# leekwoon/nav-gym

Measured on AMD Instinct MI355X. Metric: env steps/sec (whole node), 4096 envs x 1081-beam lidar, higher is better.
Workload: dtype f32

## Files before the change

### nav-gym_amd/csrc/kernels_step.hpp

```cpp

struct StepShared {
    double rp[3];
    double old_rp[3];
    double act[2];
    float lx, ly, lth;
    int steps_now;
    double cT, sT;
    int i0, j0;
    int nseg, ndisc;
    int rescan;
    int respawn;
    float t1;
    float r_all;
    unsigned long long step_key;
    unsigned long long rescan_key;
    int next_chunk;
    int park_count, park_next;
    int pair_done;
    int term;
    double wave_ratio[kMaxWaves];
};
struct PedShared {
    double *ax, *ay, *avx, *avy;
    float (*seg)[4];
    float (*disc)[2];
    float* info;
};
__host__ __device__ inline size_t ped_lds_bytes(int N) { return (size_t)144 * N + 32; }
__host__ __device__ inline size_t ped_pair_bytes(int N) { return ((size_t)(N * (N - 1) / 2 + N) * sizeof(double2) + 15) & ~(size_t)15; }
__device__ __forceinline__ PedShared ped_lds_carve(char* base, int N) {
    PedShared ps;
    double* d = (double*)base;
    ps.ax = d; ps.ay = d + (N + 1); ps.avx = d + 2 * (N + 1); ps.avy = d + 3 * (N + 1);
    float* f = (float*)(d + 4 * (N + 1));
    ps.seg = (float(*)[4])f;
    ps.disc = (float(*)[2])(f + 16 * N);
    ps.info = f + 20 * N;
    return ps;
}
struct Prims { const float (*seg)[4]; const float (*disc)[2]; float* info; };

template <int BLOCK>
__device__ __forceinline__ void finish_beams(const navsim_config& c, const StepShared& sh, const Prims pr,
                                             const double* __restrict__ tab, const float2* __restrict__ dir,
                                             const float* __restrict__ rng, float* __restrict__ rng_rw,
                                             const float* __restrict__ thr, const float* __restrict__ dthr,
                                             float* __restrict__ obs_row, int n_hist, float noise_std,
                                             uint64_t noise_key, uint64_t genv, int& crash, int& discomfort);

__device__ __forceinline__ void sfm_pair(const navsim_config& c, double xi, double yi, double vxi, double vyi,
                                         double xj, double yj, double vxj, double vyj, double& fx, double& fy) {
    fx = 0.0; fy = 0.0;
    double dxx = xj - xi, dyy = yj - yi;
    double dist = sqrt(dxx * dxx + dyy * dyy);
    if (dist < 1e-9) return;
    double ddx = dxx / dist, ddy = dyy / dist;
    double ivx = c.sfm_lambda * (vxi - vxj) + ddx;
    double ivy = c.sfm_lambda * (vyi - vyj) + ddy;
    double il = sqrt(ivx * ivx + ivy * ivy);
    if (il < 1e-9) return;
    double idx = ivx / il, idy = ivy / il;
    double theta = nv::atan2_(idx * ddy - idy * ddx, idx * ddx + idy * ddy);
    double Bq = c.sfm_gamma * il;
    double a1 = c.sfm_n_prime * Bq * theta;
    double a2 = c.sfm_n * Bq * theta;
    double fv = -nv::exp_neg(-dist / Bq - a1 * a1);
    double sgn = (theta > 0.0) ? 1.0 : ((theta < 0.0) ? -1.0 : 0.0);
    double fa = -sgn * nv::exp_neg(-dist / Bq - a2 * a2);
    fx = fv * idx + fa * (-idy);
    fy = fv * idy + fa * idx;
// ... 236 lines not shown
            if (mask_lane(inval)) raw = field.load(px, py);
            occ = (occ & ~inval) | (inval & mask_of(field.occupied(raw)));
            d = mask_sel(inval, field.decode_nz(raw, px, py), d);
        }
    } else {
        typename Field::raw_t raw = field.load(px, py);
        occ = live & mask_of(field.occupied(raw));
        d = field.decode_nz(raw, px, py);
    }
    hit |= occ;
    const float tn = t + march_step<RULE>(d);
    const lanemask_t go = live & ~occ;
    t = mask_sel(go, tn, t);
    active = go & mask_flt(tn, max_range);
}

constexpr int kIntRangeMaxSide = 1448;
__host__ __device__ __forceinline__ bool int_range_ok(int H, int W) { return H <= kIntRangeMaxSide && W <= kIntRangeMaxSide; }
__device__ __forceinline__ float hit_range_int(int ix, int iy) {
    return nv::sqrt_small_int((float)(__mul24(ix, ix) + __mul24(iy, iy)));
}
template <int RULE>
__device__ __forceinline__ float ray_result(lanemask_t hit, bool int_range, int i0, int j0, float x0, float y0, float dx, float dy,
                                            float t, float miss) {
    const int px = (int)march_pos<RULE>(x0, dx, t), py = (int)march_pos<RULE>(y0, dy, t);
    float r;
    if (int_range) {
        r = hit_range_int(px - i0, py - j0);
    } else {
        const float xd = (float)px - x0, yd = (float)py - y0;
        r = sqrtf(xd * xd + yd * yd);
    }
    return mask_sel(hit, r, miss);
}

#ifndef NAVSIM_PARK_LANES
#define NAVSIM_PARK_LANES 16
#endif
#ifndef NAVSIM_PAIR_SHARE_MIN_BLOCK
#define NAVSIM_PAIR_SHARE_MIN_BLOCK 512
#endif
constexpr int kParkLanesMax = NAVSIM_PARK_LANES;
#ifndef NAVSIM_PARK_LANES_PEDS
#define NAVSIM_PARK_LANES_PEDS 16
#endif
#ifdef NAVSIM_PARK_512
__host__ __device__ constexpr bool step_parks(int block, bool peds) { return (block == 256 && (!peds || NAVSIM_PARK_LANES_PEDS > 0)) || (block == 512 && !peds); }
#else
__host__ __device__ constexpr bool step_parks(int block, bool peds) { return block == 256 && (!peds || NAVSIM_PARK_LANES_PEDS > 0); }
#endif
__host__ __device__ inline size_t park_lds_bytes(int B, int park_lanes, bool peds) {
    return (((size_t)((B + 63) / 64) * park_lanes * (peds ? 2 : 16)) + 15) & ~(size_t)15;
}
__device__ __forceinline__ int lanes_below(lanemask_t m) {
    return (int)__builtin_amdgcn_mbcnt_hi((unsigned)(m >> 32), __builtin_amdgcn_mbcnt_lo((unsigned)m, 0u));
}

template <int BLOCK, typename Field, bool TO_LDS, int RULE, int RECT>
__device__ __forceinline__ void scan_beams_pred(const navsim_config& c, StepShared& sh,
                                                const Field& field, const uint4* __restrict__ rects,
                                                const double* __restrict__ tab,
                                                const Prims pr, float2* __restrict__ dir_lds, float* __restrict__ rng_lds,
                                                float4* __restrict__ park, const int park_lanes,
                                                const float* __restrict__ thr, const float* __restrict__ dthr,
                                                float* __restrict__ obs_row, int n_hist, float noise_std,
                                                uint64_t noise_key, uint64_t genv,
                                                int& crash, int& discomfort, bool prepare_prims = true) {
    const int B = c.n_beams, S = c.n_scan_stack, H = c.map_h, W = c.map_w;
    const float max_range = march_limit(H, W, c.range_max, c.resolution);
    const float res = (float)c.resolution;
    const float rmax = (float)c.range_max;
    const double step = nv::linspace_step(c);
    const int i0 = sh.i0, j0 = sh.j0;
    const float x0 = (float)i0, y0 = (float)j0;
    const bool int_range = int_range_ok(H, W);
    const float lx = sh.lx, ly = sh.ly;
    const int nseg = sh.nseg, ndisc = sh.ndisc;
    const unsigned uW = (unsigned)W, uH = (unsigned)H;
    const unsigned tpr = (unsigned)((W + 7) >> kRectShift);
    const float t1 = sh.t1, r_all = sh.r_all;
    const uint64_t nkey = (noise_std > 0.0f) ? nv::noise_stream(c.seed, genv, noise_key) : 0;
    int cr = 0, dc = 0;
    auto finish = [&](int k, float dx, float dy, float rr) {
        if (TO_LDS) {
            rng_lds[k] = rr * res;
            dir_lds[k] = make_float2(dx, dy);
            return;
        }
        rr = rr * res;
        for (int p = 0; p < nseg; ++p)
            nv::seg_merge(rr, lx, ly, dx, dy, pr.seg[p][0], pr.seg[p][1], pr.seg[p][2], pr.seg[p][3]);
        for (int p = 0; p < ndisc; ++p)
            nv::circle_merge(rr, lx, ly, dx, dy, pr.disc[p][0], pr.disc[p][1], nv::kLegRadius);
        rr = rr < 0.0f ? 0.0f : rr;
        rr = rr > rmax ? rmax : rr;
        if (noise_std > 0.0f && rr != rmax)
            rr = rr + noise_std * nv::gauss_noise(nkey, (uint32_t)k);
        cr |= (rr < thr[k]);
        dc |= (rr < dthr[k]);
        obs_row[(size_t)(S - 1) * B + k] = rr;
        for (int j = 0; j < S - 1; ++j)
            if (S - 1 - j > n_hist) obs_row[(size_t)j * B + k] = rr;
    };
    const float miss = (r_all >= 0.0f) ? r_all : max_range;
    if constexpr (TO_LDS) { if (prepare_prims) prims_prepare<BLOCK>(c, sh, pr); }
    constexpr bool kPark = step_parks(BLOCK, TO_LDS);
    int own_chunk = 0;
    const int lane = (int)threadIdx.x & 63;
    for (;;) {
        int chunk = 0;
        if (BLOCK > 64) {
            if (lane == 0) chunk = atomicAdd(&sh.next_chunk, 1);
            chunk = __builtin_amdgcn_readfirstlane(chunk);
        } else {
            chunk = own_chunk++;
        }
        if (chunk * 64 >= B) break;
        const int k = chunk * 64 + lane;
        const bool valid = k < B;
        float dx, dy;
        beam_dir_k(c, tab, valid ? k : B - 1, step, (double)sh.lth, sh.cT, sh.sT, dx, dy);
        float t = t1;
        lanemask_t active = mask_of(valid & (r_all < 0.0f));
        lanemask_t hit = 0;
        if constexpr (!kPark) {
            while (active != 0)
                probe_round<Field, RULE, RECT>(field, (const char*)rects, tpr, x0, y0, dx, dy, uW, uH, max_range, t, active, hit);
            if (valid) finish(k, dx, dy, ray_result<RULE>(hit, int_range, i0, j0, x0, y0, dx, dy, t, miss));
        } else {
            while ((int)__builtin_popcountll(active) > park_lanes)
                probe_round<Field, RULE, RECT>(field, (const char*)rects, tpr, x0, y0, dx, dy, uW, uH, max_range, t, active, hit);
            const bool marching = mask_lane(active);
            if (active != 0) {
                int base = 0;
                if (lane == 0) base = atomicAdd(&sh.park_count, (int)__builtin_popcountll(active));
                base = __builtin_amdgcn_readfirstlane(base);
                if (marching) {
                    if constexpr (TO_LDS) {
                        ((unsigned short*)park)[base + lanes_below(active)] = (unsigned short)k;
                        rng_lds[k] = t;
                        dir_lds[k] = make_float2(dx, dy);
                    } else {
                        park[base + lanes_below(active)] = make_float4(__int_as_float(k), t, dx, dy);
                    }
                }
            }
            if (valid & !marching) finish(k, dx, dy, ray_result<RULE>(hit, int_range, i0, j0, x0, y0, dx, dy, t, miss));
        }
    }
    if constexpr (kPark) __syncthreads();
    const int n_parked = kPark ? sh.park_count : 0;
    for (;;) {
        if (!kPark || n_parked == 0) break;
        int g = 0;
        if (lane == 0) g = atomicAdd(&sh.park_next, 64);
        g = __builtin_amdgcn_readfirstlane(g);
        if (g >= n_parked) break;
        const bool valid = g + lane < n_parked;
        int k;
        float t, dx, dy;
        if constexpr (TO_LDS) {
            k = (int)((const unsigned short*)park)[valid ? g + lane : g];
            t = rng_lds[k];
            const float2 d = dir_lds[k];
            dx = d.x; dy = d.y;
        } else {
            const float4 r = park[valid ? g + lane : g];
            k = __float_as_int(r.x);
            t = r.y; dx = r.z; dy = r.w;
        }
        lanemask_t active = mask_of(valid);
        lanemask_t hit = 0;
        while (active != 0)
            probe_round<Field, RULE, RECT>(field, (const char*)rects, tpr, x0, y0, dx, dy, uW, uH, max_range, t, active, hit);
        if (valid) finish(k, dx, dy, ray_result<RULE>(hit, int_range, i0, j0, x0, y0, dx, dy, t, miss));
    }
    if (TO_LDS) {
        __syncthreads();
        finish_beams<BLOCK>(c, sh, pr, tab, dir_lds, rng_lds, rng_lds, thr, dthr, obs_row, n_hist, noise_std,
                            noise_key, genv, cr, dc);
    }
    crash = cr;
    discomfort = dc;
}

__device__ __forceinline__ int ped_pop_waypoints(const double* wp, int head, int nw, const double (&pp)[3]) {
    while (head + 1 < nw) {
        double ddx = pp[0] - wp[2 * head], ddy = pp[1] - wp[2 * head + 1];
        if (sqrt(ddx * ddx + ddy * ddy) < 1.0) ++head;
        else break;
    }
    return head;
}
__device__ __forceinline__ void ped_pair_index(int t, int n, int& i, int& j) {
    const int n_pp = n * (n - 1) / 2;
    if (t < n_pp) {
        i = 0;
        int rem = t;
        while (rem >= n - 1 - i) { rem -= n - 1 - i; ++i; }
        j = i + 1 + rem;
    } else {
        i = t - n_pp; j = n;
    }
}
__device__ __forceinline__ void ped_pair_term(const navsim_config& c, const PedShared& ps, double2* pair, int n, int t) {
    int i, j;
    ped_pair_index(t, n, i, j);
    double fx, fy;
    sfm_pair(c, ps.ax[i], ps.ay[i], ps.avx[i], ps.avy[i], ps.ax[j], ps.ay[j], ps.avx[j], ps.avy[j], fx, fy);
    pair[t] = make_double2(fx, fy);
}
template <typename Field>
__device__ __forceinline__ void ped_sfm_step(const navsim_config& c, const Field& field, const PedShared& ps,
                                             const double2* pair, int n, int i, double vpref, const double* wp, double dt,
                                             double (&pp)[3], double (&pvel)[2]) {
    double ex = wp[0] - ps.ax[i], ey = wp[1] - ps.ay[i];
    double L = sqrt(ex * ex + ey * ey);
    if (L > 1e-9) { ex = ex / L; ey = ey / L; } else { ex = 0.0; ey = 0.0; }
    double fdx = (vpref * ex - ps.avx[i]) / c.sfm_tau;
    double fdy = (vpref * ey - ps.avy[i]) / c.sfm_tau;
    double fsx = 0.0, fsy = 0.0;
    {
        int slot = i - 1;
        for (int j = 0; j < i; ++j) {
            const double2 f = pair[slot];
            fsx -= f.x;
            fsy -= f.y;
            slot += n - 2 - j;
        }
        slot = i * (n - 1) - i * (i - 1) / 2;
        for (int j = i + 1; j < n; ++j, ++slot) {
            const double2 f = pair[slot];
            fsx += f.x;
// ... 520 lines not shown
            }
        }
        const double th = th_old + a1 * dt;
        const double th_new = reset_only ? th_old : nv::mod_2pi(th);
        const float lth = (float)th_new;
        const double ang = (l0 == 0) ? th_old : ((l0 == 1) ? th : (double)lth);
        double sn, cs;
        nv::sincos(ang, sn, cs);
        const int w0 = kPhase0Thread & 63;
        const double s0 = __shfl(sn, w0), c0 = __shfl(cs, w0), s1 = __shfl(sn, w0 + 1), c1 = __shfl(cs, w0 + 1);
        const double sT = __shfl(sn, w0 + 2), cT = __shfl(cs, w0 + 2);
        if (l0 == 0) {
            sh.old_rp[0] = rp_g[0]; sh.old_rp[1] = rp_g[1]; sh.old_rp[2] = th_old;
            sh.nseg = 0; sh.ndisc = 0; sh.rescan = 0; sh.respawn = 0; sh.term = 0;
            if constexpr (INSTALL) {
                if (pending && !in->lone) {
                    if (in->late) in->late[e] = 0;
                    if (in->late_next) in->late_next[e] = 0;
                    if (in->late_prev && in->late_prev[e]) {
                        sh.respawn = 4;
                        stage_request(in->stage.episode, in->mark, e, st.episode[e] + 1);
                        if (st.counters) atomicAdd(&st.counters[NAVSIM_COUNTER_REGEN_LATE], 1ull);
                    } else if (in->ready) {
                        const bool lng = c.regen_min_steps <= 0 || st.done_steps[e] >= c.regen_min_steps;
                        const bool rdy = stage_ready(in->ready, e) == (long long)st.episode[e];
                        if (lng && rdy) sh.respawn = 3;
                        else {
                            if (lng && in->late) in->late[e] = 1;
                            stage_request(in->stage.episode, in->mark, e, st.episode[e] + 1);
                        }
                        if (st.counters)
                            atomicAdd(&st.counters[lng ? (rdy ? NAVSIM_COUNTER_REGEN_SERVED : NAVSIM_COUNTER_REGEN_LATE) : NAVSIM_COUNTER_REGEN_SHORT], 1ull);
                    }
                }
            }
            if (!reset_only) {
                const int64_t steps_now = st.steps[e] + 1;
                st.steps[e] = steps_now;
                sh.steps_now = (int)steps_now;
                sh.act[0] = a0; sh.act[1] = a1;
                double p[3] = {sh.old_rp[0], sh.old_rp[1], sh.old_rp[2]};
                nv::set_vel_with(p, a0, a1, dt, c.axle_offset, s0, c0, s1, c1, nullptr);
                sh.rp[0] = p[0]; sh.rp[1] = p[1]; sh.rp[2] = p[2];
            } else {
                sh.rp[0] = sh.old_rp[0]; sh.rp[1] = sh.old_rp[1]; sh.rp[2] = sh.old_rp[2];
            }
            sh.lx = (float)sh.rp[0]; sh.ly = (float)sh.rp[1]; sh.lth = (float)sh.rp[2];
            nv::xy_to_ij_f32(sh.lx, sh.ly, c, sh.i0, sh.j0);
            sh.sT = sT; sh.cT = cT;
            first_probe<RULE>(field, sh.i0, sh.j0, (float)((long long)c.map_h * c.map_w), sh.t1, sh.r_all);
            sh.step_key = (unsigned long long)st.episode[e] * 0x100000000ULL +
                          (unsigned long long)(reset_only ? 0 : st.steps[e]) * 2ULL;
            sh.rescan_key = sh.step_key + 1;
            sh.next_chunk = 0; sh.park_count = 0; sh.park_next = 0; sh.pair_done = 0;
        }
    }
    __syncthreads();
    if constexpr (INSTALL) {
        if (pending && sh.respawn == 3) {
            install_arena<BLOCK>(c, st, io, *in, e, obs_row);
            install_publish(*in, st, e);
            return;
        }
        if (pending && sh.respawn == 4) return;
    }

    NAVSIM_STAMP(1);
    if constexpr (PEDS) {
        double2* pair = (double2*)(dyn_lds + ((dyn_lds_bytes + 15u) & ~15u) + ((ped_lds_bytes(N) + 15) & ~(size_t)15));
#ifdef NAVSIM_PAIR_SHARE_ALL
        constexpr int kPairWaves = (BLOCK >= NAVSIM_PAIR_SHARE_MIN_BLOCK) ? 4 : 1;
#else
        constexpr int kPairWaves = (INSTALL && BLOCK >= NAVSIM_PAIR_SHARE_MIN_BLOCK) ? 4 : 1;
#endif
        const bool pair_shared = PINL && kPairWaves > 1 && ped_advance && c.ped_model == NAVSIM_PED_SFM;
        if constexpr (PINL && kPairWaves > 1) {
            if (pair_shared && tid < kPairWaves * 64) ped_pair_share(c, ps, pair, n, tid, kPairWaves, &sh.pair_done);
        }
        if (tid < 64) {
            const int lane = tid;
            if constexpr (PINL) {
                if (ped_advance)
                    ped_advance_wave<Field>(c, st, field, e, n, lane, is_ped, pq, dt, genv, (uint64_t)st.steps[e], ps, pair,
                                            ped_head, ped_nw, pp, pvel, &sh.pair_done, pair_shared ? kPairWaves : 1);
            }
            if (reset_only && is_ped) {
                st.ped_dist[pq * 3] = 0.0; st.ped_dist[pq * 3 + 1] = 0.0; st.ped_dist[pq * 3 + 2] = 0.0;
                st.ped_prev_yaw[pq] = nv::wrap_pi(pp[2]);
            }
            if (is_ped) {
                float dist3[3];
                if (reset_only) { dist3[0] = dist3[1] = dist3[2] = 0.0f; }
                else { dist3[0] = (float)st.ped_dist[pq * 3]; dist3[1] = (float)st.ped_dist[pq * 3 + 1];
                       dist3[2] = (float)st.ped_dist[pq * 3 + 2]; }
                if (st.ped_has_legs[pq] && c.lidar_legs) {
                    float cc[4];
                    nv::leg_centres((float)pp[0], (float)pp[1], (float)pp[2], dist3[0], dist3[1], dist3[2], cc);
                    int q = atomicAdd(&sh.ndisc, 2);
                    ps.disc[q][0] = cc[0]; ps.disc[q][1] = cc[1];
                    ps.disc[q + 1][0] = cc[2]; ps.disc[q + 1][1] = cc[3];
                } else {
                    const double fpx[4] = {0.22, -0.22, -0.22, 0.22};
                    const double fpy[4] = {0.19, 0.19, -0.19, -0.19};
                    double s, cs;
                    nv::sincos(pp[2], s, cs);
                    float vx[4], vy[4];
#pragma unroll
                    for (int v = 0; v < 4; ++v) {
                        vx[v] = (float)((cs * fpx[v] - s * fpy[v]) + pp[0]);
                        vy[v] = (float)((s * fpx[v] + cs * fpy[v]) + pp[1]);
                    }
                    int q = atomicAdd(&sh.nseg, 4);
#pragma unroll
                    for (int v = 0; v < 4; ++v) {
                        int w = (v + 1) & 3;
                        ps.seg[q + v][0] = vx[v]; ps.seg[q + v][1] = vy[v];
                        ps.seg[q + v][2] = vx[w]; ps.seg[q + v][3] = vy[w];
                    }
                }
            }
            wave_lds_sync();
            prims_prepare<64>(c, sh, prims);
        }
    }

    NAVSIM_STAMP(2);
    if (kMarchPrio == 2 || base_prio == 2) __builtin_amdgcn_s_setprio(2);
    else if (base_prio == 1) __builtin_amdgcn_s_setprio(1);
    else __builtin_amdgcn_s_setprio(0);
    int n_hist = reset_only ? 0 : st.n_hist[e];
    int crash = 0, discomfort = 0;
    const uint64_t step_key = sh.step_key;
    float4* park = (float4*)dyn_lds;
    char* scan_lds = dyn_lds + park_lds_bytes(B, park_lanes, PEDS);
    float2* dir_lds = (float2*)scan_lds;
    float* rng_lds = (float*)(scan_lds + sizeof(float2) * (size_t)B);
    scan_beams_pred<BLOCK, Field, PEDS, RULE, RECT>(c, sh, field, rects, st.beam_table, prims, dir_lds, rng_lds, park, park_lanes, st.scan_threshold,
                                                         st.scan_discomfort, obs_row, n_hist, noise_std, step_key, genv, crash, discomfort, false);

    NAVSIM_STAMP(3);
    bool restart_next = false;
    if (!reset_only) {
        crash = __syncthreads_or(crash);
        discomfort = __syncthreads_or(discomfort);
        double rmin = 1.0e300;
        if (discomfort && !crash) {
            for (int k = tid; k < B; k += BLOCK)
            {
                double ratio = nv::discomfort_ratio((double)obs_row[(size_t)(S - 1) * B + k],
                                                    st.scan_threshold[k], st.scan_discomfort[k]);
                rmin = ratio < rmin ? ratio : rmin;
            }
            rmin = wave_min_f64(rmin);
            if ((tid & 63) == 0) sh.wave_ratio[tid >> 6] = rmin;
            __syncthreads();
        }
        NAVSIM_STAMP(4);
        if (tid == 0) {
            if (discomfort && !crash)
                for (int w = 1; w < (BLOCK + 63) / 64; ++w) rmin = sh.wave_ratio[w] < rmin ? sh.wave_ratio[w] : rmin;
            double prev_xy[2] = {pv_g[0], pv_g[1]};
            double pose[2] = {sh.rp[0], sh.rp[1]};
            double vel[2] = {pa_g[0], pa_g[1]};
            double goal[2] = {goal_g[0], goal_g[1]};
            nv::RewardOut o = nv::reward_scalar(c, prev_xy, pose, vel, goal, crash != 0, discomfort != 0, rmin);
            if constexpr (kFeat) {
                if (c.max_episode_steps > 0) {
                    const bool trunc = !o.done && sh.steps_now >= c.max_episode_steps;
                    if (io.truncated) io.truncated[e] = (uint8_t)trunc;
                    if (trunc) o.done = 1;
                }
            }
            io.reward[e] = o.reward;
            io.done[e] = (uint8_t)o.done;
            if constexpr (INSTALL) { if (in->late) in->late[e] = 0; if (in->late_next) in->late_next[e] = 0; }
            io.is_success[e] = o.success;
            io.is_crash[e] = o.crash;
            io.distance[e] = o.distance;
            const bool restart = o.done && c.auto_reset != NAVSIM_AUTORESET_NONE && c.n_spawn > 0;
            if (restart && c.auto_reset == NAVSIM_AUTORESET_SAME_STEP) {
                if (kFeat && io.final_obs) {
                    const bool crashed = o.crash != 0.0f;
                    const double tx = crashed ? pv_g[0] : sh.rp[0], ty = crashed ? pv_g[1] : sh.rp[1];
                    const double tyaw = nv::wrap_pi(crashed ? pv_g[2] : sh.rp[2]);
                    float* ft = io.final_obs + (size_t)e * D + (size_t)S * B;
                    ft[0] = (float)pv_g[0]; ft[1] = (float)pv_g[1];
                    ft[2] = (float)tx; ft[3] = (float)ty;
                    ft[4] = (float)pa_g[0]; ft[5] = (float)pa_g[1];
                    ft[6] = (float)tyaw;
                    if (io.final_goals) {
                        float* fg = io.final_goals + 4 * (size_t)e;
                        fg[0] = (float)tx; fg[1] = (float)ty; fg[2] = (float)goal_g[0]; fg[3] = (float)goal_g[1];
                    }
                    sh.term = crashed ? 2 : 1;
                }
                uint64_t h = nv::hash4(c.seed, genv, (uint64_t)st.episode[e], 0x5eedULL);
                int idx = (int)(h % (uint64_t)c.n_spawn);
                const double* sp = st.spawn_pose + ((size_t)e * c.n_spawn + idx) * 3;
                const double* sg = st.spawn_goal + ((size_t)e * c.n_spawn + idx) * 2;
                sh.rp[0] = sp[0]; sh.rp[1] = sp[1]; sh.rp[2] = sp[2];
                goal_g[0] = sg[0]; goal_g[1] = sg[1];
#ifndef NAVSIM_DIAG_NO_DONE_STEPS
                if (st.done_steps) st.done_steps[e] = sh.steps_now;
#endif
                st.episode[e] += 1;
                st.steps[e] = 0;
                sh.rescan_key = (unsigned long long)st.episode[e] * 0x100000000ULL;
                sh.respawn = 1; sh.rescan = c.defer_reset_scan ? 0 : 1;
                if constexpr (INSTALL) if (in->ready) {
                    const bool lng = c.regen_min_steps <= 0 || st.done_steps[e] >= c.regen_min_steps;
                    const bool rdy = stage_ready(in->ready, e) == (long long)st.episode[e];
                    if (lng && rdy) { sh.respawn = 3; sh.rescan = 0; }
                    else if (lng && in->late) in->late[e] = 1;
                    if (st.counters)
                        atomicAdd(&st.counters[lng ? (rdy ? NAVSIM_COUNTER_REGEN_SERVED : NAVSIM_COUNTER_REGEN_LATE) : NAVSIM_COUNTER_REGEN_SHORT], 1ull);
                    if (!(lng && rdy)) stage_request(in->stage.episode, in->mark, e, st.episode[e] + 1);
                }
            } else {
                restart_next = kFeat && restart;
                if (o.crash != 0.0f) {
                    sh.rp[0] = pv_g[0]; sh.rp[1] = pv_g[1]; sh.rp[2] = pv_g[2];
                    sh.rescan = 1;
                }
            }
#ifdef NAVSIM_DIAG_NO_RESCAN
            sh.rescan = 0;
#endif
            if constexpr (!kFeat) {
                if (sh.rescan) {
                    sh.next_chunk = 0; sh.park_count = 0; sh.park_next = 0;
                    sh.lx = (float)sh.rp[0]; sh.ly = (float)sh.rp[1]; sh.lth = (float)sh.rp[2];
                    nv::xy_to_ij_f32(sh.lx, sh.ly, c, sh.i0, sh.j0);
                    nv::sincos((double)sh.lth, sh.sT, sh.cT);
                    first_probe<RULE>(field, sh.i0, sh.j0, (float)((long long)c.map_h * c.map_w), sh.t1, sh.r_all);
                }
            }
        }
        __syncthreads();
        if constexpr (!kFeat) {
            if (sh.rescan) {
                if (sh.respawn) n_hist = 0;
                int c2, d2;
                scan_beams_pred<BLOCK, Field, PEDS, RULE, RECT>(c, sh, field, rects, st.beam_table, prims, dir_lds, rng_lds, park, park_lanes, st.scan_threshold,
                                                                     st.scan_discomfort, obs_row, n_hist, noise_std, sh.rescan_key, genv, c2, d2);
            }
        } else {
            float* final_row = io.final_obs ? io.final_obs + (size_t)e * D : nullptr;
            const int term = sh.term;
            if (term == 1) {
                for (int j = 0; j < S; ++j) {
                    const bool old = j < S - 1 && S - 1 - j <= n_hist;
                    for (int k = tid; k < B; k += BLOCK)
                        final_row[(size_t)j * B + k] = old ? obs_prev[(size_t)(j + 1) * B + k] : obs_row[(size_t)(S - 1) * B + k];
                }
                __syncthreads();
            }
            for (int pass = (term == 2) ? 0 : 1; pass < 2; ++pass) {
                if (pass == 1 && !sh.rescan) break;
                if (tid == 0) {
                    const double* at = (pass == 0) ? pv_g : sh.rp;
                    sh.next_chunk = 0; sh.park_count = 0; sh.park_next = 0;
                    sh.lx = (float)at[0]; sh.ly = (float)at[1]; sh.lth = (float)at[2];
                    nv::xy_to_ij_f32(sh.lx, sh.ly, c, sh.i0, sh.j0);
                    nv::sincos((double)sh.lth, sh.sT, sh.cT);
                    first_probe<RULE>(field, sh.i0, sh.j0, (float)((long long)c.map_h * c.map_w), sh.t1, sh.r_all);
                }
                __syncthreads();
                if (pass == 1 && sh.respawn) n_hist = 0;
                int c2, d2;
                scan_beams_pred<BLOCK, Field, PEDS, RULE, RECT>(c, sh, field, rects, st.beam_table, prims, dir_lds, rng_lds, park, park_lanes, st.scan_threshold,
                                                                     st.scan_discomfort, pass == 0 ? final_row : obs_row, n_hist, noise_std,
                                                                     pass == 0 ? step_key + 1 : sh.rescan_key, genv, c2, d2);
                if (pass == 0) {
                    for (int j = 0; j < S - 1; ++j)
                        if (S - 1 - j <= n_hist)
                            for (int k = tid; k < B; k += BLOCK) final_row[(size_t)j * B + k] = obs_prev[(size_t)(j + 1) * B + k];
                    __syncthreads();
                }
            }
        }
    }

    NAVSIM_STAMP(5);
    if (kMarchPrio != 0 && base_prio < kMarchPrio) {
        if (base_prio == 1) __builtin_amdgcn_s_setprio(1);
        else __builtin_amdgcn_s_setprio(0);
    }
    const bool fresh = reset_only || sh.respawn;
    if (!fresh && obs_prev) {
        for (int j = 0; j < S - 1; ++j)
            if (S - 1 - j <= n_hist)
                for (int k = tid; k < B; k += BLOCK) obs_row[(size_t)j * B + k] = obs_prev[(size_t)(j + 1) * B + k];
    }
    if (tid == 0) {
        float* tail = obs_row + (size_t)S * B;
        double yaw = nv::wrap_pi(sh.rp[2]);
        double pxy0 = fresh ? sh.rp[0] : pv_g[0];
        double pxy1 = fresh ? sh.rp[1] : pv_g[1];
        double v0 = fresh ? 0.0 : pa_g[0], v1 = fresh ? 0.0 : pa_g[1];
        tail[0] = (float)pxy0; tail[1] = (float)pxy1;
        tail[2] = (float)sh.rp[0]; tail[3] = (float)sh.rp[1];
        tail[4] = (float)v0; tail[5] = (float)v1;
        tail[6] = (float)yaw;
        if (io.achieved_goal) { io.achieved_goal[2 * e] = (float)sh.rp[0]; io.achieved_goal[2 * e + 1] = (float)sh.rp[1]; }
        if (io.desired_goal) { io.desired_goal[2 * e] = (float)goal_g[0]; io.desired_goal[2 * e + 1] = (float)goal_g[1]; }
        rp_g[0] = sh.rp[0]; rp_g[1] = sh.rp[1]; rp_g[2] = sh.rp[2];
        if (fresh) { pa_g[0] = 0.0; pa_g[1] = 0.0; st.n_hist[e] = (S - 1 < 1) ? S - 1 : 1; }
        else       { pa_g[0] = sh.act[0]; pa_g[1] = sh.act[1]; st.n_hist[e] = (n_hist + 1 < S - 1) ? n_hist + 1 : S - 1; }
        if (reset_only) st.steps[e] = 0;
        pv_g[0] = sh.rp[0]; pv_g[1] = sh.rp[1]; pv_g[2] = yaw;
        if (restart_next) {
            uint64_t h = nv::hash4(c.seed, genv, (uint64_t)st.episode[e], 0x5eedULL);
            int idx = (int)(h % (uint64_t)c.n_spawn);
            const double* sp = st.spawn_pose + ((size_t)e * c.n_spawn + idx) * 3;
            const double* sg = st.spawn_goal + ((size_t)e * c.n_spawn + idx) * 2;
            rp_g[0] = sp[0]; rp_g[1] = sp[1]; rp_g[2] = sp[2];
            goal_g[0] = sg[0]; goal_g[1] = sg[1];
            if (st.done_steps) st.done_steps[e] = sh.steps_now;
            st.episode[e] += 1;
            st.steps[e] = 0;
            if constexpr (INSTALL) {
                if (in->late_next && in->ready) {
                    const bool lng = c.regen_min_steps <= 0 || sh.steps_now >= c.regen_min_steps;
// ... 191 lines not shown
```

### nav-gym_amd/csrc/navsim_step_inst.hip

```cpp
#include "preamble.hpp"

#if !defined(NAVSIM_INST_BLOCK) || !defined(NAVSIM_INST_PEDS)
#error "compile with -DNAVSIM_INST_BLOCK=64|256|512|1024 -DNAVSIM_INST_PEDS=0|1 (csrc/Makefile)"
#endif

namespace {
#include "kernels_field.hpp"
#include "kernels_rect.hpp"
#include "kernels_plan.hpp"
#include "kernels_regen_dev.hpp"
#include "kernels_step.hpp"
}
#include "step_plan.hpp"

namespace {

template <typename Kernel, typename... Args>
int launch(Kernel kernel, const StepLaunch& l, int blocks, int block, size_t lds, const Args&... args) {
    if (allow_lds((const void*)kernel, lds) != NAVSIM_OK) return NAVSIM_E_UNSUPPORTED;
    if (l.prepare_only) return NAVSIM_OK;
    kernel<<<blocks, block, lds, l.stream>>>(args...);
    return NAVSIM_OK;
}

template <int BLOCK, bool PEDS, typename Field, int RECT, int RULE, bool PINL>
int launch_step_pinl(const navsim_config* c, const navsim_state* st, const navsim_step_io* io, const StepLaunch& l, const StepPlan& p) {
    constexpr bool kPacked = !std::is_same<Field, FieldF32>::value;
    const unsigned scan = (unsigned)step_lds_scan_bytes(c, p.park);
    const int blocks = l.grid > 0 ? l.grid : c->n_envs;
    if constexpr (PEDS && PINL) {
        if (l.part == kStepPartReplan) {
            const size_t pl = plan_lds(c->map_h / 5, c->map_w / 5), lds = p.lds > pl ? p.lds : pl;
            if (l.install) {
                if constexpr (kPacked)
                    return launch(navsim_step_replan_install_kernel<BLOCK, Field, RULE, RECT>, l, l.grid + c->n_envs, BLOCK, lds,
                                  *c, *st, *io, *l.install, scan, p.park, p.rect_off, l.grid, l.max_queries);
                return NAVSIM_E_UNSUPPORTED;
            }
            return launch(navsim_step_replan_kernel<BLOCK, Field, RULE, RECT>, l, l.grid + c->n_envs, BLOCK, lds,
                          *c, *st, *io, scan, p.park, p.rect_off, l.grid, l.max_queries);
        }
        if (l.part == NAVSIM_STEP_DUE)
            return launch(navsim_step_due_kernel<BLOCK, Field, RULE, RECT>, l, blocks, BLOCK, p.lds, *c, *st, *io, scan, p.park, p.rect_off);
    }
    if constexpr (PINL == PEDS && kPacked) {
        if (l.install)
            return launch(navsim_step_install_kernel<BLOCK, PEDS, Field, RULE, RECT>, l, blocks, BLOCK, p.lds,
                          *c, *st, *io, *l.install, step_kernel_word(l), l.mask, scan, p.park, p.rect_off);
    }
    if (l.install) return NAVSIM_E_UNSUPPORTED;
    if constexpr (!PEDS) {
        const bool feat = io->final_obs || io->reset_mask || c->auto_reset == NAVSIM_AUTORESET_NEXT_STEP ||
                          (c->max_episode_steps > 0 && !l.reset_only);
        if (!feat)
            return launch(navsim_step_kernel<BLOCK, PEDS, Field, RULE, RECT, PINL, false>, l, blocks, BLOCK, p.lds,
                          *c, *st, *io, step_kernel_word(l), l.mask, scan, p.park, p.rect_off);
    }
    return launch(navsim_step_kernel<BLOCK, PEDS, Field, RULE, RECT, PINL, true>, l, blocks, BLOCK, p.lds,
                  *c, *st, *io, step_kernel_word(l), l.mask, scan, p.park, p.rect_off);
}
template <int BLOCK, bool PEDS, typename Field, int RECT, int RULE>
int launch_step_kernel(const navsim_config* c, const navsim_state* st, const navsim_step_io* io, const StepLaunch& l, const StepPlan& p) {
    if constexpr (PEDS) {
        if ((!l.reset_only && !l.peds_done) || l.install) return launch_step_pinl<BLOCK, PEDS, Field, RECT, RULE, true>(c, st, io, l, p);
    }
    return launch_step_pinl<BLOCK, PEDS, Field, RECT, RULE, false>(c, st, io, l, p);
}

template <int BLOCK, bool PEDS, typename Field, int RECT>
int launch_step_rule(const navsim_config* c, const navsim_state* st, const navsim_step_io* io, const StepLaunch& l,
                     const StepPlan& p) {
    return with_march_rule<Field>(march_rule_variant(c), [&](auto rule) {
        return launch_step_kernel<BLOCK, PEDS, Field, RECT, decltype(rule)::value>(c, st, io, l, p);
    });
}

template <int BLOCK, bool PEDS, typename Field>
int launch_step_field(const navsim_config* c, const navsim_state* st, const navsim_step_io* io, const StepLaunch& l,
                      const StepPlan& p) {
    if (p.rect == 2) return launch_step_rule<BLOCK, PEDS, Field, 2>(c, st, io, l, p);
    return p.rect ? launch_step_rule<BLOCK, PEDS, Field, 1>(c, st, io, l, p)
// ... 34 lines not shown
```

### nav-gym_amd/csrc/step_plan.hpp

```cpp

struct StepPlan {
    int block;
    int rect;
    int park;
    size_t lds;
    unsigned rect_off;
};
struct StepLaunch {
    bool reset_only = false;
    bool peds_done = false;
    int part = NAVSIM_STEP_ALL;
    const uint8_t* mask = nullptr;
    int grid = 0;
    int max_queries = 0;
    const StepInstall* install = nullptr;
    bool prepare_only = false;
    hipStream_t stream = nullptr;
};

namespace {
constexpr size_t kLdsPerCu = 160 * 1024;
int allow_lds(const void* kernel, size_t lds) {
    if (lds <= 64 * 1024) return NAVSIM_OK;
    if (lds > kLdsPerCu) return NAVSIM_E_UNSUPPORTED;
    struct Granted { const void* kernel; int device; size_t lds; };
    constexpr int kSlots = 256;
    static Granted table[kSlots];
    static int used = 0;
    static std::mutex lock;
    int dev = 0;
    if (hipGetDevice(&dev) != hipSuccess) dev = -1;
    std::lock_guard<std::mutex> guard(lock);
    Granted* slot = nullptr;
    for (int i = 0; i < used; ++i)
        if (table[i].kernel == kernel && table[i].device == dev) { slot = &table[i]; break; }
    if (slot && slot->lds >= lds) return NAVSIM_OK;
    if (hipFuncSetAttribute(kernel, hipFuncAttributeMaxDynamicSharedMemorySize, (int)lds) != hipSuccess) return NAVSIM_E_UNSUPPORTED;
    if (!slot && used < kSlots) { slot = &table[used++]; slot->kernel = kernel; slot->device = dev; }
    if (slot) slot->lds = lds;
    return NAVSIM_OK;
}

int device_cu_count() {
    static std::atomic<int> cache[64];
    int dev = 0;
    if (hipGetDevice(&dev) != hipSuccess || dev < 0 || dev >= 64) return 256;
    int v = cache[dev].load(std::memory_order_relaxed);
    if (v > 0) return v;
    int n = 0;
    if (hipDeviceGetAttribute(&n, hipDeviceAttributeMultiprocessorCount, dev) != hipSuccess || n <= 0) n = 256;
    cache[dev].store(n, std::memory_order_relaxed);
    return n;
}

int step_park_lanes(const navsim_config* c, int block) {
    const bool peds = c->ped_model != NAVSIM_PED_NONE;
    if (!step_parks(block, peds)) return 0;
    if (peds) return c->n_beams <= 65535 ? NAVSIM_PARK_LANES_PEDS : 0;
    return kParkLanesMax;
}
size_t step_lds_scan_bytes(const navsim_config* c, int park_lanes) {
    const bool peds = c->ped_model != NAVSIM_PED_NONE;
    return park_lds_bytes(c->n_beams, park_lanes, peds) + (peds ? (size_t)c->n_beams * (sizeof(float2) + sizeof(float)) : 0);
}
size_t ped_update_lds_bytes(const navsim_config* c) {
    return (size_t)ped_pack(c->max_peds) * ped_slot_bytes(c->max_peds);
}
bool ped_split_on(const navsim_config* c) {
    if (c->ped_model == NAVSIM_PED_NONE || ped_update_lds_bytes(c) > 64 * 1024) return false;
    return c->ped_split == 2;
}
size_t step_lds_bytes(const navsim_config* c, int park_lanes) {
    size_t lds = step_lds_scan_bytes(c, park_lanes);
    if (c->ped_model != NAVSIM_PED_NONE) {
        lds = ((lds + 15) & ~(size_t)15) + ped_lds_bytes(c->max_peds);
        if (!ped_split_on(c)) lds = ((lds + 15) & ~(size_t)15) + ped_pair_bytes(c->max_peds);
    }
    return lds;
}

int pick_step_block(const navsim_config* c) {
    if (c->step_block) return c->step_block;
    const int B = c->n_beams;
    const long cus = device_cu_count();
    if (B <= 64) return 64;
    if ((long)c->n_envs >= 12 * cus || B <= 256) return 256;
    if ((long)c->n_envs > 2 * cus || B <= 512) return 512;
    return 1024;
}

int march_rule_variant(const navsim_config* c) {
    if (c->march_rule == NAVSIM_MARCH_F32 || c->march_rule == NAVSIM_MARCH_F32_FMA) return c->march_rule;
    const int side = c->map_h > c->map_w ? c->map_h : c->map_w;
    return (c->field_format == NAVSIM_FIELD_U16T && side <= 1448) ? kMarchF64Exact32 : NAVSIM_MARCH_F64;
}
template <typename Field, typename F>
int with_march_rule(int rule, F&& f) {
#ifdef NAVSIM_ONLY_RULE
    if (rule != NAVSIM_ONLY_RULE) return NAVSIM_E_UNSUPPORTED;
    return f(std::integral_constant<int, NAVSIM_ONLY_RULE>{});
#else
    switch (rule) {
        case NAVSIM_MARCH_F32: return f(std::integral_constant<int, NAVSIM_MARCH_F32>{});
        case NAVSIM_MARCH_F32_FMA: return f(std::integral_constant<int, NAVSIM_MARCH_F32_FMA>{});
        case kMarchF64Exact32:
            if constexpr (!std::is_same<Field, FieldF32>::value) return f(std::integral_constant<int, kMarchF64Exact32>{});
            [[fallthrough]];
        default: return f(std::integral_constant<int, NAVSIM_MARCH_F64>{});
    }
#endif
}

int step_kernel_word(const StepLaunch& l) {
    return (l.reset_only ? kStepWordResetOnly : 0) | ((l.peds_done ? 1 : 0) << kStepWordPedsDoneBit) | (l.part << kStepWordPartShift);
}
StepPlan plan_step(const navsim_config* c, const navsim_state* st, int grid = 0) {
    StepPlan p;
    p.block = pick_step_block(c);
    p.rect = st->rect_table ? 1 : 0;
    p.park = step_park_lanes(c, p.block);
    p.lds = step_lds_bytes(c, p.park);
    p.rect_off = 0;
    if (p.rect && st->rect_index && c->closed_maps && c->rect_lds != 1 && c->field_format == NAVSIM_FIELD_U16T) {
        const size_t row = rect_index_row_bytes(c->map_h, c->map_w);
        const size_t base = (p.lds + 15) & ~(size_t)15;
        const size_t total = base + row + 1024;
        const int per_cu = p.block >= 1024 ? 2 : (p.block == 512 ? 4 : 5);
        const bool lone = grid > 0 && grid <= device_cu_count();
        const bool fits = c->rect_lds == 2 || lone ? total <= kLdsPerCu : (size_t)per_cu * total <= kLdsPerCu;
        if (fits) { p.rect = 2; p.lds = base + row; p.rect_off = (unsigned)row; }
    }
    return p;
}
}
```

Before: 51.13 million.

## Add second park level for long rays and dense finish pass in scan

When more than 64 rays are parked, the parked-ray march now parks a second time once a wave has at most 12 active lanes. The leftover long rays go into a second LDS buffer and are marched in a final level. This repacks straggler rays into fuller waves and cuts divergent probe rounds. In the no-pedestrian parking path, per-beam finishing (clamp, noise, thresholds, obs writes) is also moved into a separate dense pass over LDS ranges, so the finish work no longer runs on scattered lanes. The cost is extra LDS, extra barriers, more atomics, and a diagnostic model script.

Result: slower. 48.41 million (-5.3%).

```diff
diff --git a/nav-gym_amd/csrc/kernels_step.hpp b/nav-gym_amd/csrc/kernels_step.hpp
--- a/nav-gym_amd/csrc/kernels_step.hpp
+++ b/nav-gym_amd/csrc/kernels_step.hpp
@@ -16,6 +16,8 @@
     unsigned long long rescan_key;
     int next_chunk;
     int park_count, park_next;
+    int repark_count, repark_next;
+    int finish_next;
     int pair_done;
     int term;
     double wave_ratio[kMaxWaves];
@@ -358,6 +360,24 @@
 __host__ __device__ inline size_t park_lds_bytes(int B, int park_lanes, bool peds) {
     return (((size_t)((B + 63) / 64) * park_lanes * (peds ? 2 : 16)) + 15) & ~(size_t)15;
 }
+#ifndef NAVSIM_REPARK_LANES
+#define NAVSIM_REPARK_LANES 12
+#endif
+constexpr int kReparkLanes = NAVSIM_REPARK_LANES;
+__host__ __device__ inline size_t repark_lds_bytes(int B, int park_lanes, bool peds) {
+    const size_t groups = ((size_t)((B + 63) / 64) * park_lanes + 63) / 64;
+    return ((groups * kReparkLanes * (peds ? 2 : 16)) + 15) & ~(size_t)15;
+}
+struct ScanLds { size_t park2, dir, rng, end; };
+__host__ __device__ constexpr bool scan_dense_finish(int block, bool peds) { return !peds && step_parks(block, false); }
+__host__ __device__ inline ScanLds scan_lds_layout(int B, int park_lanes, bool peds, bool dense) {
+    ScanLds l;
+    l.park2 = park_lds_bytes(B, park_lanes, peds);
+    l.dir = l.park2 + repark_lds_bytes(B, park_lanes, peds);
+    l.rng = l.dir + (peds ? sizeof(float2) * (size_t)B : 0);
+    l.end = l.rng + ((peds || dense) ? sizeof(float) * (size_t)B : 0);
+    return l;
+}
 __device__ __forceinline__ int lanes_below(lanemask_t m) {
     return (int)__builtin_amdgcn_mbcnt_hi((unsigned)(m >> 32), __builtin_amdgcn_mbcnt_lo((unsigned)m, 0u));
 }
@@ -367,7 +387,7 @@
                                                 const Field& field, const uint4* __restrict__ rects,
                                                 const double* __restrict__ tab,
                                                 const Prims pr, float2* __restrict__ dir_lds, float* __restrict__ rng_lds,
-                                                float4* __restrict__ park, const int park_lanes,
+                                                float4* __restrict__ park, float4* __restrict__ park2, const int park_lanes,
                                                 const float* __restrict__ thr, const float* __restrict__ dthr,
                                                 float* __restrict__ obs_row, int n_hist, float noise_std,
                                                 uint64_t noise_key, uint64_t genv,
@@ -385,9 +405,15 @@
     const unsigned uW = (unsigned)W, uH = (unsigned)H;
     const unsigned tpr = (unsigned)((W + 7) >> kRectShift);
     const float t1 = sh.t1, r_all = sh.r_all;
-    const uint64_t nkey = (noise_std > 0.0f) ? nv::noise_stream(c.seed, genv, noise_key) : 0;
+    constexpr bool kPark = step_parks(BLOCK, TO_LDS);
+    constexpr bool kDense = scan_dense_finish(BLOCK, TO_LDS);
+    const uint64_t nkey = (!kDense && noise_std > 0.0f) ? nv::noise_stream(c.seed, genv, noise_key) : 0;
     int cr = 0, dc = 0;
     auto finish = [&](int k, float dx, float dy, float rr) {
+        if constexpr (kDense) {
+            rng_lds[k] = rr;
+            return;
+        }
         if (TO_LDS) {
             rng_lds[k] = rr * res;
             dir_lds[k] = make_float2(dx, dy);
@@ -410,7 +436,6 @@
     };
     const float miss = (r_all >= 0.0f) ? r_all : max_range;
     if constexpr (TO_LDS) { if (prepare_prims) prims_prepare<BLOCK>(c, sh, pr); }
-    constexpr bool kPark = step_parks(BLOCK, TO_LDS);
     int own_chunk = 0;
     const int lane = (int)threadIdx.x & 63;
     for (;;) {
@@ -454,37 +479,80 @@
             if (valid & !marching) finish(k, dx, dy, ray_result<RULE>(hit, int_range, i0, j0, x0, y0, dx, dy, t, miss));
         }
     }
-    if constexpr (kPark) __syncthreads();
-    const int n_parked = kPark ? sh.park_count : 0;
-    for (;;) {
-        if (!kPark || n_parked == 0) break;
-        int g = 0;
-        if (lane == 0) g = atomicAdd(&sh.park_next, 64);
-        g = __builtin_amdgcn_readfirstlane(g);
-        if (g >= n_parked) break;
-        const bool valid = g + lane < n_parked;
-        int k;
-        float t, dx, dy;
-        if constexpr (TO_LDS) {
-            k = (int)((const unsigned short*)park)[valid ? g + lane : g];
-            t = rng_lds[k];
-            const float2 d = dir_lds[k];
-            dx = d.x; dy = d.y;
-        } else {
-            const float4 r = park[valid ? g + lane : g];
-            k = __float_as_int(r.x);
-            t = r.y; dx = r.z; dy = r.w;
-        }
-        lanemask_t active = mask_of(valid);
-        lanemask_t hit = 0;
-        while (active != 0)
-            probe_round<Field, RULE, RECT>(field, (const char*)rects, tpr, x0, y0, dx, dy, uW, uH, max_range, t, active, hit);
-        if (valid) finish(k, dx, dy, ray_result<RULE>(hit, int_range, i0, j0, x0, y0, dx, dy, t, miss));
+    for (int level = 0; kPark && level < 2; ++level) {
+        __syncthreads();
+        const int n_parked = level ? sh.repark_count : sh.park_count;
+        const int stop = (kReparkLanes > 0 && level == 0 && n_parked > 64) ? kReparkLanes : 0;
+        const float4* from = level ? park2 : park;
+        int* next = level ? &sh.repark_next : &sh.park_next;
+        for (;;) {
+            if (n_parked == 0) break;
+            int g = 0;
+            if (lane == 0) g = atomicAdd(next, 64);
+            g = __builtin_amdgcn_readfirstlane(g);
+            if (g >= n_parked) break;
+            const bool valid = g + lane < n_parked;
+            int k;
+            float t, dx, dy;
+            if constexpr (TO_LDS) {
+                k = (int)((const unsigned short*)from)[valid ? g + lane : g];
+                t = rng_lds[k];
+                const float2 d = dir_lds[k];
+                dx = d.x; dy = d.y;
+            } else {
+                const float4 r = from[valid ? g + lane : g];
+                k = __float_as_int(r.x);
+                t = r.y; dx = r.z; dy = r.w;
+            }
+            lanemask_t active = mask_of(valid);
+            lanemask_t hit = 0;
+            while ((int)__builtin_popcountll(active) > stop)
+                probe_round<Field, RULE, RECT>(field, (const char*)rects, tpr, x0, y0, dx, dy, uW, uH, max_range, t, active, hit);
+            const bool marching = mask_lane(active);
+            if (active != 0) {
+                int base = 0;
+                if (lane == 0) base = atomicAdd(&sh.repark_count, (int)__builtin_popcountll(active));
+                base = __builtin_amdgcn_readfirstlane(base);
+                if (marching) {
+                    if constexpr (TO_LDS) {
+                        ((unsigned short*)park2)[base + lanes_below(active)] = (unsigned short)k;
+                        rng_lds[k] = t;
+                    } else {
+                        park2[base + lanes_below(active)] = make_float4(__int_as_float(k), t, dx, dy);
+                    }
+                }
+            }
+            if (valid & !marching) finish(k, dx, dy, ray_result<RULE>(hit, int_range, i0, j0, x0, y0, dx, dy, t, miss));
+        }
+        if (stop == 0) break;
     }
     if (TO_LDS) {
         __syncthreads();
         finish_beams<BLOCK>(c, sh, pr, tab, dir_lds, rng_lds, rng_lds, thr, dthr, obs_row, n_hist, noise_std,
                             noise_key, genv, cr, dc);
+    }
+    if constexpr (kDense) {
+        __syncthreads();
+        const uint64_t fkey = (noise_std > 0.0f) ? nv::noise_stream(c.seed, genv, noise_key) : 0;
+        for (;;) {
+            int chunk = 0;
+            if (lane == 0) chunk = atomicAdd(&sh.finish_next, 1);
+            chunk = __builtin_amdgcn_readfirstlane(chunk);
+            if (chunk * 64 >= B) break;
+            const int k = chunk * 64 + lane;
+            if (k < B) {
+                float rr = rng_lds[k] * res;
+                rr = rr < 0.0f ? 0.0f : rr;
+                rr = rr > rmax ? rmax : rr;
+                if (noise_std > 0.0f && rr != rmax)
+                    rr = rr + noise_std * nv::gauss_noise(fkey, (uint32_t)k);
+                cr |= (rr < thr[k]);
+                dc |= (rr < dthr[k]);
+                obs_row[(size_t)(S - 1) * B + k] = rr;
+                for (int j = 0; j < S - 1; ++j)
+                    if (S - 1 - j > n_hist) obs_row[(size_t)j * B + k] = rr;
+            }
+        }
     }
     crash = cr;
     discomfort = dc;
@@ -1111,7 +1179,7 @@
             sh.step_key = (unsigned long long)st.episode[e] * 0x100000000ULL +
                           (unsigned long long)(reset_only ? 0 : st.steps[e]) * 2ULL;
             sh.rescan_key = sh.step_key + 1;
-            sh.next_chunk = 0; sh.park_count = 0; sh.park_next = 0; sh.pair_done = 0;
+            sh.next_chunk = 0; sh.park_count = 0; sh.park_next = 0; sh.repark_count = 0; sh.repark_next = 0; sh.finish_next = 0; sh.pair_done = 0;
         }
     }
     __syncthreads();
@@ -1190,11 +1258,12 @@
     int n_hist = reset_only ? 0 : st.n_hist[e];
     int crash = 0, discomfort = 0;
     const uint64_t step_key = sh.step_key;
+    const ScanLds scan_at = scan_lds_layout(B, park_lanes, PEDS, scan_dense_finish(BLOCK, PEDS));
     float4* park = (float4*)dyn_lds;
-    char* scan_lds = dyn_lds + park_lds_bytes(B, park_lanes, PEDS);
-    float2* dir_lds = (float2*)scan_lds;
-    float* rng_lds = (float*)(scan_lds + sizeof(float2) * (size_t)B);
-    scan_beams_pred<BLOCK, Field, PEDS, RULE, RECT>(c, sh, field, rects, st.beam_table, prims, dir_lds, rng_lds, park, park_lanes, st.scan_threshold,
+    float4* park2 = (float4*)(dyn_lds + scan_at.park2);
+    float2* dir_lds = (float2*)(dyn_lds + scan_at.dir);
+    float* rng_lds = (float*)(dyn_lds + scan_at.rng);
+    scan_beams_pred<BLOCK, Field, PEDS, RULE, RECT>(c, sh, field, rects, st.beam_table, prims, dir_lds, rng_lds, park, park2, park_lanes, st.scan_threshold,
                                                          st.scan_discomfort, obs_row, n_hist, noise_std, step_key, genv, crash, discomfort, false);
 
     NAVSIM_STAMP(3);
@@ -1287,7 +1356,7 @@
 #endif
             if constexpr (!kFeat) {
                 if (sh.rescan) {
-                    sh.next_chunk = 0; sh.park_count = 0; sh.park_next = 0;
+                    sh.next_chunk = 0; sh.park_count = 0; sh.park_next = 0; sh.repark_count = 0; sh.repark_next = 0; sh.finish_next = 0;
                     sh.lx = (float)sh.rp[0]; sh.ly = (float)sh.rp[1]; sh.lth = (float)sh.rp[2];
                     nv::xy_to_ij_f32(sh.lx, sh.ly, c, sh.i0, sh.j0);
                     nv::sincos((double)sh.lth, sh.sT, sh.cT);
@@ -1300,7 +1369,7 @@
             if (sh.rescan) {
                 if (sh.respawn) n_hist = 0;
                 int c2, d2;
-                scan_beams_pred<BLOCK, Field, PEDS, RULE, RECT>(c, sh, field, rects, st.beam_table, prims, dir_lds, rng_lds, park, park_lanes, st.scan_threshold,
+                scan_beams_pred<BLOCK, Field, PEDS, RULE, RECT>(c, sh, field, rects, st.beam_table, prims, dir_lds, rng_lds, park, park2, park_lanes, st.scan_threshold,
                                                                      st.scan_discomfort, obs_row, n_hist, noise_std, sh.rescan_key, genv, c2, d2);
             }
         } else {
@@ -1318,7 +1387,7 @@
                 if (pass == 1 && !sh.rescan) break;
                 if (tid == 0) {
                     const double* at = (pass == 0) ? pv_g : sh.rp;
-                    sh.next_chunk = 0; sh.park_count = 0; sh.park_next = 0;
+                    sh.next_chunk = 0; sh.park_count = 0; sh.park_next = 0; sh.repark_count = 0; sh.repark_next = 0; sh.finish_next = 0;
                     sh.lx = (float)at[0]; sh.ly = (float)at[1]; sh.lth = (float)at[2];
                     nv::xy_to_ij_f32(sh.lx, sh.ly, c, sh.i0, sh.j0);
                     nv::sincos((double)sh.lth, sh.sT, sh.cT);
@@ -1327,7 +1396,7 @@
                 __syncthreads();
                 if (pass == 1 && sh.respawn) n_hist = 0;
                 int c2, d2;
-                scan_beams_pred<BLOCK, Field, PEDS, RULE, RECT>(c, sh, field, rects, st.beam_table, prims, dir_lds, rng_lds, park, park_lanes, st.scan_threshold,
+                scan_beams_pred<BLOCK, Field, PEDS, RULE, RECT>(c, sh, field, rects, st.beam_table, prims, dir_lds, rng_lds, park, park2, park_lanes, st.scan_threshold,
                                                                      st.scan_discomfort, pass == 0 ? final_row : obs_row, n_hist, noise_std,
                                                                      pass == 0 ? step_key + 1 : sh.rescan_key, genv, c2, d2);
                 if (pass == 0) {
diff --git a/nav-gym_amd/csrc/navsim_step_inst.hip b/nav-gym_amd/csrc/navsim_step_inst.hip
--- a/nav-gym_amd/csrc/navsim_step_inst.hip
+++ b/nav-gym_amd/csrc/navsim_step_inst.hip
@@ -26,7 +26,7 @@
 template <int BLOCK, bool PEDS, typename Field, int RECT, int RULE, bool PINL>
 int launch_step_pinl(const navsim_config* c, const navsim_state* st, const navsim_step_io* io, const StepLaunch& l, const StepPlan& p) {
     constexpr bool kPacked = !std::is_same<Field, FieldF32>::value;
-    const unsigned scan = (unsigned)step_lds_scan_bytes(c, p.park);
+    const unsigned scan = (unsigned)step_lds_scan_bytes(c, BLOCK, p.park);
     const int blocks = l.grid > 0 ? l.grid : c->n_envs;
     if constexpr (PEDS && PINL) {
         if (l.part == kStepPartReplan) {
diff --git a/nav-gym_amd/csrc/step_plan.hpp b/nav-gym_amd/csrc/step_plan.hpp
--- a/nav-gym_amd/csrc/step_plan.hpp
+++ b/nav-gym_amd/csrc/step_plan.hpp
@@ -59,9 +59,9 @@
     if (peds) return c->n_beams <= 65535 ? NAVSIM_PARK_LANES_PEDS : 0;
     return kParkLanesMax;
 }
-size_t step_lds_scan_bytes(const navsim_config* c, int park_lanes) {
+size_t step_lds_scan_bytes(const navsim_config* c, int block, int park_lanes) {
     const bool peds = c->ped_model != NAVSIM_PED_NONE;
-    return park_lds_bytes(c->n_beams, park_lanes, peds) + (peds ? (size_t)c->n_beams * (sizeof(float2) + sizeof(float)) : 0);
+    return scan_lds_layout(c->n_beams, park_lanes, peds, scan_dense_finish(block, peds)).end;
 }
 size_t ped_update_lds_bytes(const navsim_config* c) {
     return (size_t)ped_pack(c->max_peds) * ped_slot_bytes(c->max_peds);
@@ -70,8 +70,8 @@
     if (c->ped_model == NAVSIM_PED_NONE || ped_update_lds_bytes(c) > 64 * 1024) return false;
     return c->ped_split == 2;
 }
-size_t step_lds_bytes(const navsim_config* c, int park_lanes) {
-    size_t lds = step_lds_scan_bytes(c, park_lanes);
+size_t step_lds_bytes(const navsim_config* c, int block, int park_lanes) {
+    size_t lds = step_lds_scan_bytes(c, block, park_lanes);
     if (c->ped_model != NAVSIM_PED_NONE) {
         lds = ((lds + 15) & ~(size_t)15) + ped_lds_bytes(c->max_peds);
         if (!ped_split_on(c)) lds = ((lds + 15) & ~(size_t)15) + ped_pair_bytes(c->max_peds);
@@ -119,7 +119,7 @@
     p.block = pick_step_block(c);
     p.rect = st->rect_table ? 1 : 0;
     p.park = step_park_lanes(c, p.block);
-    p.lds = step_lds_bytes(c, p.park);
+    p.lds = step_lds_bytes(c, p.block, p.park);
     p.rect_off = 0;
     if (p.rect && st->rect_index && c->closed_maps && c->rect_lds != 1 && c->field_format == NAVSIM_FIELD_U16T) {
         const size_t row = rect_index_row_bytes(c->map_h, c->map_w);
diff --git a/profiles/_diag/park_cascade_model.py b/profiles/_diag/park_cascade_model.py
--- /dev/null
+++ b/profiles/_diag/park_cascade_model.py
@@ -0,0 +1,110 @@
+import argparse
+import os
+import sys
+
+import numpy as np
+from scipy import ndimage
+
+ROOT = os.path.join(os.path.dirname(os.path.abspath(__file__)), "..", "..")
+sys.path.insert(0, os.path.join(ROOT, "nav-gym_amd"))
+from nav_gym_amd import world
+
+B = 1081
+ANG = np.linspace(-0.75 * np.pi, 0.75 * np.pi, B)
+RESOLUTION, RANGE_MAX = 0.05, 25.0
+KERNEL = ("16", "12*")
+
+
+def probe_counts(d, i0, j0, th):
+    size = d.shape[0]
+    limit = min(np.floor(RANGE_MAX / RESOLUTION) + 4.0, float(size * size))
+    dx, dy = np.cos(th + ANG), np.sin(th + ANG)
+    t = np.full(B, max(0.999 * d[i0, j0], 1.0))
+    n = np.zeros(B, int)
+    act = np.full(B, t[0] < limit)
+    while act.any():
+        x = np.clip((i0 + t * dx).astype(int), 0, size - 1); y = np.clip((j0 + t * dy).astype(int), 0, size - 1)
+        dd = d[x, y]
+        n += act
+        act &= dd > 0
+        t = np.where(act, t + np.maximum(0.999 * dd, 1.0), t)
+        act &= t < limit
+    return n
+
+
+def leave(v, T):
+    v = np.asarray(v)
+    if T <= 0 or len(v) <= T:
+        return (int(v.max()) if len(v) else 0), []
+    s = np.sort(v)[::-1]
+    r = int(s[T])
+    return r, [int(x - r) for x in v if x > r]
+
+
+def run(n, sched):
+    rounds = groups = 0
+    pool = []
+    for c0 in range(0, B, 64):
+        r, rem = leave(n[c0:c0 + 64], int(sched[0].rstrip("*")))
+        rounds += r; groups += 1; pool += rem
+    parked, levels, last = len(pool), 0, 0
+    level = 1
+    while pool:
+        spec = sched[level] if level < len(sched) else (sched[-1] if sched[-1].endswith("*") else "0")
+        T = int(spec.rstrip("*"))
+        if spec.endswith("*") and len(pool) <= 64:
+            T = 0
+        nxt = []
+        for q in range(0, len(pool), 64):
+            r, rem = leave(pool[q:q + 64], T)
+            rounds += r; groups += 1; nxt += rem
+            last = len(pool[q:q + 64])
+        pool = nxt; levels += 1; level += 1
+    return rounds, groups, parked, levels, last
+
+
+def poses_of(occ, per_map, rng):
+    for e in range(occ.shape[0]):
+        d = ndimage.distance_transform_edt(occ[e] == 0)
+        free = np.argwhere(d > 0)
+        for i0, j0 in free[rng.choice(len(free), per_map, replace=False)]:
+            yield d, int(i0), int(j0), float(np.float32(rng.uniform(-np.pi, np.pi)))
+
+
+def main():
+    ap = argparse.ArgumentParser()
+    ap.add_argument("--schedule", action="append", default=[], help="thresholds per level, e.g. 16,12* or 32,24,16*")
+    ap.add_argument("--world", nargs=3, type=int, metavar=("SIZE", "SEED", "MAPS"))
+    a = ap.parse_args()
+    rng = np.random.default_rng(0)
+    if a.world:
+        size, seed, maps = a.world
+        occ = world.make_maps(maps, size, seed)
+        per_map = -(-200 // maps)
+        rows = [run(probe_counts(*p), KERNEL) for p in poses_of(occ, per_map, rng)][:200]
+        parked = np.array([r[2] for r in rows]); levels = np.array([r[3] for r in rows]); last = np.array([r[4] for r in rows])
+        print("make_maps(%d, %d, %d), %d free poses, 1081 beams, chunks park at %s, parked groups at %s" % (maps, size, seed, len(rows), KERNEL[0], KERNEL[1].rstrip("*")))
+        print("rays parked by the chunks per scan: min %d, mean %.1f, max %d; scans with more than 64: %d of %d"
+              % (parked.min(), parked.mean(), parked.max(), int((parked > 64).sum()), len(rows)))
+        print("levels behind the chunks: %s" % {int(k): int(v) for k, v in zip(*np.unique(levels, return_counts=True))})
+        print("scans whose last group holds fewer than 64 rays: %d; its size: min %d, mean %.1f"
+              % (int(((last < 64) & (last > 0)).sum()), last[last > 0].min(), last[last > 0].mean()))
+        return
+    occ = world.make_maps(48, 500, 1234)
+    counts = [probe_counts(*p) for p in poses_of(occ, 2, rng)]
+    table = [("64 adjacent beams, no parking", ["0"]), ("park at 16, parked rays run to the end", ["16"]),
+             ("park at 16, parked groups re-park at 16 until at most 64 rays are left", ["16", "16*"]),
+             ("same, thresholds 16 / 24 / 16", ["16", "24", "16*"]), ("park at 32, then 16", ["32", "16*"]),
+             ("park at 32, then 24, then 16", ["32", "24", "16*"]),
+             ("the kernel: park at 16, more than 64 parked: groups re-park at 12, then to the end", list(KERNEL))]
+    table += [("--schedule " + s, s.split(",")) for s in a.schedule]
+    print("%d scans, %.2f probes per ray" % (len(counts), np.mean([c.mean() for c in counts])))
+    print("%-86s %12s %16s" % ("schedule", "rounds/scan", "groups + chunks"))
+    for name, sched in table:
+        res = np.array([run(c, sched)[:2] for c in counts], float).mean(axis=0)
+        print("%-86s %12.1f %16.1f" % (name, res[0], res[1]))
+    print("%-86s %12.1f" % ("perfect packing (bound)", np.mean([c.sum() / 64.0 for c in counts])))
+
+
+if __name__ == "__main__":
+    main()
```
